# DarlingHang/st-nerf

Measured on NVIDIA H100. Metric: rays/sec, higher is better.
Workload: dtype f32 via fp16x3 split products (wgmma), f32 accumulate

## Files before the change

### st-nerf_b200/csrc/api.cu

```cuda
#include <algorithm>
#include <new>
#include <stdlib.h>
#include <string.h>
#include <vector>
#include "common.cuh"
#include "mlp_tc.cuh"

namespace stnerf {
thread_local char g_cuda_err[512] = "";
std::atomic<unsigned long long> g_launches{0};
}

using namespace stnerf;

namespace {

struct SpaceNetDev {
  float* blob = nullptr;
  SpaceNetW w{};
  TcNet tc{};
  bool loaded = false;
};
struct MotionNetDev {
  float* blob = nullptr;
// ... 4 lines not shown

}

struct stnerf_ctx {
  stnerf_model_desc desc{};
  int l = 0, num_sms = 0, device = 0, precision = 0, chunk_rays = 65536;
  SpaceNetDev space[2][STNERF_MAX_LAYERS];
  MotionNetDev motion[STNERF_MAX_LAYERS];
  stnerf_scene scene{};
  DevScene dscene{};
  bool have_scene = false;
  int cap_n1 = 0, cap_s2 = 0;
  long long last_chunk_rays = 0;
  int last_n1 = 0, last_s2 = 0;
  bool last_reuse = false;
  float *t_coarse = nullptr, *raw_coarse = nullptr, *t_fine = nullptr, *raw_fine = nullptr, *xyz = nullptr;
  float *xyz_coarse = nullptr, *z_new = nullptr;
  uint8_t* src_map = nullptr;
  bool no_reuse = false;
  float* cbuf = nullptr;
  uint8_t* mask_ws = nullptr;
  int *hit = nullptr, *counts = nullptr, *lerp_flags = nullptr;
  size_t ws_bytes = 0;
  float *h_rays = nullptr, *h_out = nullptr;
  uint8_t* h_mask = nullptr;
  size_t h_rays_bytes = 0, h_out_bytes = 0, h_mask_bytes = 0;
  float *v_rays = nullptr, *v_img[2] = {nullptr, nullptr};
  size_t v_rays_bytes = 0, v_img_bytes[2] = {0, 0};
  cudaStream_t copy_in = nullptr, copy_out = nullptr;
  std::vector<cudaEvent_t> ev_pool;
  float* box_table = nullptr;
  int box_frames = 0;
  bool no_fuse = false;
  int* any_frac = nullptr;
  RayIdMap idmap{0, 0, 0};
  int rot_mode[STNERF_MAX_LAYERS] = {0};
  float rot_R[STNERF_MAX_LAYERS][9] = {}, rot_c[STNERF_MAX_LAYERS][3] = {};
  struct ProfRec { int cls; cudaEvent_t a, b; double points; int count_slot; int S; };
  bool prof_on = false;
  std::vector<ProfRec> prof;
  int* prof_counts = nullptr;
  int prof_chunks = 0;
};

namespace {
constexpr int PROF_MAX_CHUNKS = 1 << 16;
struct ProfScope {
  stnerf_ctx* c; int idx = -1; cudaStream_t st;
  ProfScope(stnerf_ctx* c_, int cls, double points, int count_slot, int S, cudaStream_t st_) : c(c_), st(st_) {
    if (!c->prof_on) return;
    stnerf_ctx::ProfRec r{cls, nullptr, nullptr, points, count_slot, S};
    if (cudaEventCreate(&r.a) != cudaSuccess || cudaEventCreate(&r.b) != cudaSuccess) return;
    cudaEventRecord(r.a, st);
    c->prof.push_back(r);
    idx = (int)c->prof.size() - 1;
  }
  ~ProfScope() { if (idx >= 0) cudaEventRecord(c->prof[idx].b, st); }
};
}

static void free_ws(stnerf_ctx* c) {
  cudaFree(c->t_coarse); cudaFree(c->raw_coarse); cudaFree(c->t_fine); cudaFree(c->raw_fine); cudaFree(c->xyz);
  cudaFree(c->xyz_coarse); cudaFree(c->z_new); cudaFree(c->src_map);
  c->xyz_coarse = c->z_new = nullptr; c->src_map = nullptr;
  cudaFree(c->cbuf); c->cbuf = nullptr;
  cudaFree(c->mask_ws); cudaFree(c->hit); cudaFree(c->counts); cudaFree(c->lerp_flags);
// ... 53 lines not shown
    case STNERF_OK: return "ok";
    case STNERF_EINVAL: return "invalid argument";
    case STNERF_ENODEVICE: return "no usable CUDA device (needs sm_90)";
    case STNERF_ECUDA: return "CUDA runtime error (see stnerf_last_cuda_error)";
    case STNERF_ENOWEIGHTS: return "network weights not loaded";
    case STNERF_ENOMEM: return "out of device memory";
    default: return "unknown error";
  }
}
const char* stnerf_last_cuda_error(void) { return g_cuda_err; }
uint64_t stnerf_launch_count(void) { return g_launches.load(); }

int stnerf_create(stnerf_handle* out, const stnerf_model_desc* d) {
  if (!out || !d || d->n_layers < 2 || d->n_layers > STNERF_MAX_LAYERS) return STNERF_EINVAL;
  if (d->precision < 0 || d->precision > STNERF_PREC_TC_3XF16_CF || d->chunk_rays < 0) return STNERF_EINVAL;
  if ((long long)d->chunk_rays * STNERF_MAX_S >= (1LL << 31)) return STNERF_EINVAL;
  int ndev = 0;
  if (cudaGetDeviceCount(&ndev) != cudaSuccess || ndev == 0) { cudaGetLastError(); return STNERF_ENODEVICE; }
  int dev = 0;
  STNERF_CUDA(cudaGetDevice(&dev));
  cudaDeviceProp prop;
  STNERF_CUDA(cudaGetDeviceProperties(&prop, dev));
  if (prop.major != 9 || prop.minor != 0) return STNERF_ENODEVICE;
  stnerf_ctx* c = new (std::nothrow) stnerf_ctx();
  if (!c) return STNERF_ENOMEM;
  c->desc = *d;
  c->l = d->n_layers;
  c->device = dev;
  c->num_sms = prop.multiProcessorCount;
  c->precision = d->precision;
  c->chunk_rays = d->chunk_rays > 0 ? d->chunk_rays : 65536;
  if (const char* e = getenv("STNERF_NO_FUSE")) c->no_fuse = (e[0] == '1');
  if (const char* e = getenv("STNERF_NO_REUSE")) c->no_reuse = (e[0] == '1');
  if (cudaMalloc((void**)&c->any_frac, 4) != cudaSuccess) { delete c; return STNERF_ENOMEM; }
  *out = c;
  return STNERF_OK;
}

void stnerf_destroy(stnerf_handle c) {
  if (!c) return;
  cudaDeviceSynchronize();
  free_ws(c);
  for (int f = 0; f < 2; ++f)
    for (int i = 0; i < STNERF_MAX_LAYERS; ++i) { cudaFree(c->space[f][i].blob); tc_free(c->space[f][i].tc); }
  for (int i = 0; i < STNERF_MAX_LAYERS; ++i) { cudaFree(c->motion[i].blob); tc_free(c->motion[i].tc); }
  cudaFree(c->h_rays); cudaFree(c->h_out); cudaFree(c->h_mask); cudaFree(c->any_frac);
  cudaFree(c->v_rays); cudaFree(c->v_img[0]); cudaFree(c->v_img[1]); cudaFree(c->box_table);
  if (c->copy_in) cudaStreamDestroy(c->copy_in);
  if (c->copy_out) cudaStreamDestroy(c->copy_out);
  for (cudaEvent_t e : c->ev_pool) cudaEventDestroy(e);
  if (c->prof_counts) cudaFreeHost(c->prof_counts);
  delete c;
}

int stnerf_set_precision(stnerf_handle c, int precision) {
  if (!c || precision < 0 || precision > STNERF_PREC_TC_3XF16_CF) return STNERF_EINVAL;
  c->precision = precision;
  return STNERF_OK;
}

int stnerf_reserve(stnerf_handle c, int n1, int n2) {
  if (!c || n1 < 3 || n1 > STNERF_MAX_N1 || n2 < 0 || n1 + n2 > STNERF_MAX_S) return STNERF_EINVAL;
  return ensure_ws(c, n1, n1 + n2);
}
size_t stnerf_workspace_bytes(stnerf_handle c) { return c ? c->ws_bytes : 0; }

// ... 246 lines not shown
    if (n > 0 && cap > 0) STNERF_CUDA(cudaMallocAsync((void**)&buf, (size_t)n * cap * stride * sizeof(float), st));
    return STNERF_OK;
  }
  int rotate(const float* rays, long long m, LayerRays& lr) {
    for (int i = 0; i < STNERF_MAX_LAYERS; ++i) lr.p[i] = rays;
    for (int k = 0; k < n; ++k) {
      float* dst = buf + (size_t)k * cap * stride;
      const int rc = launch_rotate_rays(rays, m, stride, rot[k], dst, st);
      if (rc) return rc;
      lr.p[layer[k]] = dst;
    }
    return STNERF_OK;
  }
  ~RotatedRays() { if (buf) cudaFreeAsync(buf, st); }
};

static void fill_edit(PointSrc& s, const stnerf_scene& sc, int layer, bool fine) {
  s.shift_on = sc.shift_on[layer];
  s.scale_on = fine ? sc.scale_fine_on[layer] : sc.scale_coarse_on[layer];
  for (int a = 0; a < 3; ++a) { s.shift[a] = sc.shift[layer][a]; s.pivot[a] = sc.pivot[a]; }
  s.scale = sc.scale[layer];
  if (!s.scale_on) s.scale = 1.0f;
}

static int run_spacenet(stnerf_ctx* c, const PointSrc& src, SpaceNetDev& net, float* raw, float* rgb, float* sigma,
                        cudaStream_t st, int count_slot = -1, const FuseCoarse* fuse = nullptr, bool fine_pass = false) {
  if (!net.loaded) return STNERF_ENOWEIGHTS;
  ProfScope ps(c, 0, (double)src.n_slots * src.S, count_slot, src.S, st);
  if (c->precision == STNERF_PREC_FP32_SIMT)
    return launch_spacenet_simt(src, net.w, raw, 0, rgb, sigma, c->num_sms, st);
  if (src.mode == SRC_EXPLICIT) {
    float* cb = nullptr;
    STNERF_CUDA(cudaMallocAsync((void**)&cb, (size_t)std::max<long long>(src.n_slots, 1) * 128 * sizeof(float), st));
    const int rc = tc_launch_spacenet(src, net.tc, c->precision, cb, raw, rgb, sigma, c->num_sms, st, nullptr, fine_pass);
    STNERF_CUDA(cudaFreeAsync(cb, st));
    return rc;
  }
  return tc_launch_spacenet(src, net.tc, c->precision, c->cbuf, raw, rgb, sigma, c->num_sms, st, fuse, fine_pass);
}
static int run_motionnet(stnerf_ctx* c, const PointSrc& src, MotionNetDev& net, const int* lerp_flag, int lerp_force,
                         float* xyz_out, float* flow_out, cudaStream_t st, int count_slot = -1) {
  if (!net.loaded) return STNERF_ENOWEIGHTS;
  ProfScope ps(c, 1, (double)src.n_slots * src.S, count_slot, src.S, st);
  if (c->precision == STNERF_PREC_FP32_SIMT)
    return launch_motionnet_simt(src, net.w, lerp_flag, lerp_force, xyz_out, flow_out, c->num_sms, st);
  return tc_launch_motionnet(src, net.tc, c->precision, lerp_flag, lerp_force, xyz_out, flow_out, c->num_sms, st);
}

static int run_nets(stnerf_ctx* c, const LayerRays& rays, long long n, int ray_stride, bool fine, int S, cudaStream_t st,
                    int chunk_slot, const FuseCoarse* fuse = nullptr, bool want_raw = true, float* coarse_imgs = nullptr,
                    long long plane = 0, int reuse_n1 = 0) {
  const long long R = c->chunk_rays;
  const float* tbuf = fine ? c->t_fine : c->t_coarse;
  float* rawbuf = fine ? c->raw_fine : c->raw_coarse;
  const long long tl = R * (fine ? c->cap_s2 : c->cap_n1);
  for (int i = 0; i < c->l; ++i) {
    if (i > 0 && !c->scene.shown[i]) continue;
    PointSrc s;
    memset(&s, 0, sizeof(s));
    s.mode = SRC_MARCH;
    s.rays = rays.p[i]; s.ray_stride = ray_stride;
    s.t = tbuf + i * tl;
    s.S = S; s.layer = c->scene.shared_frame_id ? 0 : i;
    s.pos_stride = 3; s.time_stride = 1;
    fill_edit(s, c->scene, i, fine);
    float* raw = want_raw ? rawbuf + (size_t)i * tl * 4 : nullptr;
    FuseCoarse f;
    memset(&f, 0, sizeof(f));
    if (fuse) {
      f = *fuse;
      f.on = 1; f.layer = i; f.is_bkgd = (i == 0);
      f.t_fine = c->t_fine + (size_t)i * R * c->cap_s2;
      f.z_new = fuse->z_new ? c->z_new + (size_t)i * R * c->cap_s2 : nullptr;
      f.src_map = fuse->z_new ? c->src_map + (size_t)i * R * c->cap_s2 : nullptr;
      f.u = fuse->u ? fuse->u + (size_t)i * fuse->n_total * fuse->n2 : nullptr;
      f.img = coarse_imgs ? coarse_imgs + (size_t)(1 + i) * plane : nullptr;
    }
    int rc;
    if (i == 0) {
// ... 863 lines not shown
```

### st-nerf_b200/csrc/mlp_tc.cu

```cuda
#include <cuda_fp16.h>
#include <string.h>
#include <type_traits>
#include <vector>
#include "mlp_tc.cuh"
#include "resample.cuh"

namespace stnerf {

namespace {

constexpr int TILE_M = 128;
constexpr int ABLOCK = 16384;
constexpr int STAGE_BYTES = 16384;
constexpr int NTHREADS = 384;
constexpr int MATH_WG0 = 1, N_MATH_WARPS = 8;
constexpr int MAX_STAGE = 8;
constexpr int REGS_WG0 = 56, REGS_MATH = 224;
static_assert(128 * REGS_WG0 + 256 * REGS_MATH <= 384 * 168, "register file");
constexpr int BAR_WFULL = 0, BAR_WEMPTY = 8, BAR_RAWFULL = 16, BAR_RAWEMPTY = 18;
constexpr int MISC_ROWS = 256;
constexpr int MISC_PART = MISC_ROWS + 128 * 24;
constexpr int MISC_CDF = MISC_PART + 2048;
constexpr int MISC_TOTAL = MISC_CDF + 512;

__device__ __forceinline__ uint32_t smem_u32(const void* p) { return (uint32_t)__cvta_generic_to_shared(p); }

__device__ __forceinline__ void mbar_init(uint32_t bar, uint32_t count) {
  asm volatile("mbarrier.init.shared::cta.b64 [%0], %1;" ::"r"(bar), "r"(count) : "memory");
}
__device__ __forceinline__ void mbar_arrive(uint32_t bar) {
  asm volatile("mbarrier.arrive.shared::cta.b64 _, [%0];" ::"r"(bar) : "memory");
}
__device__ __forceinline__ void mbar_arrive_if(uint32_t bar, bool pred) {
  asm volatile("{\n\t.reg .pred p;\n\tsetp.ne.b32 p, %1, 0;\n\t@p mbarrier.arrive.shared::cta.b64 _, [%0];\n\t}" ::"r"(bar), "r"((uint32_t)pred)
               : "memory");
}
__device__ __forceinline__ void mbar_expect_tx(uint32_t bar, uint32_t bytes) {
  asm volatile("mbarrier.arrive.expect_tx.shared::cta.b64 _, [%0], %1;" ::"r"(bar), "r"(bytes) : "memory");
}
__device__ __forceinline__ void mbar_wait(uint32_t bar, uint32_t parity) {
  asm volatile(
      "{\n\t.reg .pred p;\n\t.reg .u32 c;\n\t"
      "mov.u32 c, 0;\n"
      "WAIT_%=:\n\t"
      "mbarrier.try_wait.parity.shared::cta.b64 p, [%0], %1;\n\t"
      "@p bra.uni DONE_%=;\n\t"
      "add.u32 c, c, 1;\n\t"
      "setp.gt.u32 p, c, 67108864;\n\t"
      "@p trap;\n\t"
      "bra.uni WAIT_%=;\n"
      "DONE_%=:\n\t}" ::"r"(bar), "r"(parity)
      : "memory");
}
__device__ __forceinline__ void bulk_g2s(uint32_t dst, const void* src, uint32_t bytes, uint32_t bar) {
  asm volatile("cp.async.bulk.shared::cluster.global.mbarrier::complete_tx::bytes [%0], [%1], %2, [%3];" ::"r"(dst),
               "l"(src), "r"(bytes), "r"(bar)
               : "memory");
}
__device__ __forceinline__ void fence_proxy_async() { asm volatile("fence.proxy.async.shared::cta;" ::: "memory"); }
template <int R>
__device__ __forceinline__ void setmaxnreg_dec() { asm volatile("setmaxnreg.dec.sync.aligned.u32 %0;" ::"n"(R)); }
template <int R>
__device__ __forceinline__ void setmaxnreg_inc() { asm volatile("setmaxnreg.inc.sync.aligned.u32 %0;" ::"n"(R)); }
__device__ __forceinline__ void wg_bar_sync(int wg) { asm volatile("bar.sync %0, 128;" ::"r"(1 + wg) : "memory"); }

__device__ __forceinline__ void load_stage_elect(uint32_t dst, const void* src, uint32_t bytes, uint32_t bar) {
  asm volatile(
      "{\n\t.reg .pred pe;\n\t"
      "elect.sync _|pe, 0xffffffff;\n\t"
      "@pe mbarrier.arrive.expect_tx.shared::cta.b64 _, [%3], %2;\n\t"
      "@pe cp.async.bulk.shared::cluster.global.mbarrier::complete_tx::bytes [%0], [%1], %2, [%3];\n\t}" ::"r"(dst),
      "l"(src), "r"(bytes), "r"(bar)
      : "memory");
}

__device__ __forceinline__ uint64_t desc_sw128(uint32_t saddr) {
  return (uint64_t)((saddr >> 4) & 0x3FFF) | ((uint64_t)1 << 16) | ((uint64_t)(1024 >> 4) << 32) | ((uint64_t)1 << 62);
}
__device__ __forceinline__ uint64_t desc_sw64(uint32_t saddr) {
  return (uint64_t)((saddr >> 4) & 0x3FFF) | ((uint64_t)1 << 16) | ((uint64_t)(512 >> 4) << 32) | ((uint64_t)2 << 62);
}
__device__ __forceinline__ void wgmma_fence() { asm volatile("wgmma.fence.sync.aligned;" ::: "memory"); }
__device__ __forceinline__ void wgmma_commit() { asm volatile("wgmma.commit_group.sync.aligned;" ::: "memory"); }
template <int N>
// ... 108 lines not shown
  static constexpr int LO_STRIDE = 2 * ABLOCK;
  static constexpr int ENC_LO_STRIDE = 2 * ABLOCK;
  static constexpr int n_stage = 8, stage_bytes = 8192;
  static constexpr int ring_base = 4 * ABLOCK, misc_base = ring_base + n_stage * stage_bytes, smem_total = misc_base + MISC_TOTAL;
  __host__ __device__ static constexpr int n_out(int) { return 128; }
  __host__ __device__ static constexpr int act_chunks(int l) { return l == 0 ? 0 : 2; }
  __host__ __device__ static constexpr int enc_chunks(int l) { return l == 0 ? 2 : 0; }
  __host__ __device__ static constexpr bool enc_first(int) { return false; }
};
static_assert(Sched<NET_SPACE>::n_stage <= MAX_STAGE && Sched<NET_MOTION>::n_stage <= MAX_STAGE, "barrier slots");

enum { A_HI = 0, A_LO = 1, A_HI_LO = 2 };
template <int A>
struct WStep {
  static constexpr int a = A;
  uint32_t offset;
  uint32_t sub;
};
template <int NET>
struct WSched {
  using S = Sched<NET>;
  __host__ __device__ static constexpr int n_chunks(int l) { return S::act_chunks(l) + S::enc_chunks(l); }
  __host__ __device__ static constexpr uint32_t stage_bytes(int l) { return (uint32_t)S::n_out(l) * 64; }
  __host__ __device__ static constexpr size_t layer_bytes(int l) { return (size_t)n_chunks(l) * 2  * 2  * stage_bytes(l); }
  __host__ __device__ static constexpr int chunk_at(int l, int c) {
    return S::enc_first(l) ? (c == 0 ? S::act_chunks(l) : c - 1) : c;
  }
  static constexpr bool enc_first_valid() {
    for (int l = 0; l < S::N_LAYERS; ++l)
      if (S::enc_first(l) && (S::act_chunks(l) == 0 || S::enc_chunks(l) == 0)) return false;
    return true;
  }
  static_assert(enc_first_valid(), "enc_first(l) needs activation chunks and an encoding chunk to reorder");
  template <bool LOFIRST, class C, class F>
  __device__ __forceinline__ static void for_each_step(int l, bool split, C&& chunk, F&& f) {
    const int nact = S::act_chunks(l), nch = nact + S::enc_chunks(l);
    const uint32_t bytes = stage_bytes(l);
    auto at = [&](const auto& a, int c, uint32_t sub, uint32_t lo_stage, auto op) {
      f(a, WStep<decltype(op)::value>{(2 * (2 * (uint32_t)c + sub) + lo_stage) * bytes, sub});
    };
    using HI = std::integral_constant<int, A_HI>;
    using LO = std::integral_constant<int, A_LO>;
    using HI_LO = std::integral_constant<int, A_HI_LO>;
    if (!LOFIRST || !split) {
      for (int c = 0; c < nch; ++c) {
        const auto a = chunk(chunk_at(l, c));
        for (uint32_t sub = 0; sub < 2; ++sub) {
          if (split) { at(a, c, sub, 1u, HI()); at(a, c, sub, 0u, HI_LO()); }
          else at(a, c, sub, 0u, HI());
        }
      }
    } else {
      for (int c = 0; c < nch; ++c) {
        const auto a = chunk(chunk_at(l, c));
        for (uint32_t sub = 0; sub < 2; ++sub) { at(a, c, sub, 1u, HI()); at(a, c, sub, 0u, LO()); }
      }
      for (int c = 0; c < nch; ++c) {
        const auto a = chunk(chunk_at(l, c));
        for (uint32_t sub = 0; sub < 2; ++sub) at(a, c, sub, 0u, HI());
      }
    }
  }
};

template <int NET>
__host__ __device__ constexpr size_t stream_bytes_per_tile() {
  size_t n = 0;
  for (int l = 0; l < Sched<NET>::N_LAYERS; ++l) n += WSched<NET>::layer_bytes(l);
  return n;
}

struct TcParams {
  FuseCoarse fuse;
  PointSrc src;
  const uint8_t* wstream;
  const float* aux;
  const float* cbuf;
  int exact;
  int single_last;
  int lo_first;
  float* raw;
  float* rgb_out;
  float* sigma_out;
  float* xyz_out;
  float* flow_out;
  const int* lerp_flag;
  int lerp_force;
};

constexpr int AUX_BIAS = 0, AUX_WSIG = 8 * 256, AUX_BSIG = AUX_WSIG + 256, AUX_WOUT = AUX_BSIG + 4,
              AUX_BOUT = AUX_WOUT + 3 * 128, AUX_FLOATS = AUX_BOUT + 4;


struct Pt { float x, y, z, tm; int out_index; int cidx; };

__device__ __forceinline__ Pt fetch_pt(const PointSrc& s, long long p, long long n_points) {
  Pt q;
  q.x = q.y = q.z = q.tm = 0.f;
  q.out_index = -1;
  q.cidx = 0;
  if (p >= n_points) return q;
  if (s.mode == SRC_EXPLICIT) {
    const float* pp = s.pos + p * s.pos_stride;
    q.x = pp[0]; q.y = pp[1]; q.z = pp[2];
    if (s.times) q.tm = s.times[p * s.time_stride];
    q.out_index = (int)p;
    q.cidx = (int)p;
    return q;
  }
  const long long slot = p / s.S;
  const int k = (int)(p - slot * s.S);
  const long long ray = s.hit ? (long long)s.hit[slot] : slot;
  const float* rp = s.rays + ray * s.ray_stride;
// ... 163 lines not shown
          if (F.apply_thr && v < F.thr) v = 0.0f;
        }
        t[s] = tk;
        sg[s] = v;
      }
      const float* up = F.u ? F.u + ray * n2 : nullptr;
      const uint64_t seed = F.seed;
      const uint32_t stream = 64u + (uint32_t)F.layer;
      const unsigned long long gid = F.idmap(F.ray_base + ray);
      rs::LayerOut lo;
      rs::composite_resample_ray<2, NZ>(
          t, sg, n1, n2, F.boarder,
          [rp, lane](int s) {
            const float4 v = rp[s * 32 + lane];
            return make_float3(__fdiv_rn(1.0f, __fadd_rn(1.0f, expf(-v.x))), __fdiv_rn(1.0f, __fadd_rn(1.0f, expf(-v.y))),
                               __fdiv_rn(1.0f, __fadd_rn(1.0f, expf(-v.z))));
          },
          [up, seed, stream, gid](int jj) { return up ? up[jj] : philox_uniform(seed, stream, gid, (uint32_t)jj); },
          cdf, F.t_fine + ray * (n1 + n2), lane, lo, F.z_new ? F.z_new + ray * n2 : nullptr,
          F.z_new ? F.src_map + ray * (n1 + n2) : nullptr);
      if (F.img && lane < 5) {
        const long long rg = F.ray_base + ray;
        const float v = lane == 0 ? lo.pix[0] : lane == 1 ? lo.pix[1] : lane == 2 ? lo.pix[2] : lane == 3 ? lo.pix[3] : lo.pix[4];
        if (F.pixels) F.img[rg * 5 + lane] = v;
        else if (lane < 3) F.img[rg * 3 + lane] = v;
        else F.img[(long long)lane * F.n_total + rg] = v;
      }
    }
    __syncwarp();
    if (lane == 0) mbar_arrive(bar_empty);
  }
}

template <int NET, int N, bool LOFIRST>
__device__ __forceinline__ void mma_layer(float (&acc)[128], const uint32_t (&alo)[64], int l, bool sp, uint32_t sbase,
                                          uint32_t a_row, uint32_t bars, uint32_t& cnt, int lane) {
  using S = Sched<NET>;
  using W = WSched<NET>;
  constexpr uint32_t NST = S::n_stage;
#pragma unroll
  for (int i = 0; i < N / 2; ++i) acc[i] = 0.f;
  acc_fence<N / 2>(acc);
  wgmma_fence();
  const int nact = S::act_chunks(l);
  int pend = -1;
  auto release = [&](int s) {
    __syncwarp();
    mbar_arrive_if(bars + 8u * (uint32_t)(BAR_WEMPTY + s), lane == 0);
  };
  auto a_block = [&](int ch) {
    uint32_t hi, lo = 0;
    int z = -1;
    if (ch < nact) {
      hi = sbase + S::act_base + ch * ABLOCK + a_row;
      if constexpr (S::lo_in_regs) z = ch;
      else lo = hi + S::LO_STRIDE;
    } else {
      hi = sbase + S::enc_base + (ch - nact) * ABLOCK + a_row;
      lo = hi + S::ENC_LO_STRIDE;
    }
    return make_int3((int)hi, (int)lo, z);
  };
  W::template for_each_step<LOFIRST>(l, sp, a_block, [&](const int3& a, auto st) {
    const uint32_t hi = (uint32_t)a.x + 64u * st.sub, lo = (uint32_t)a.y + 64u * st.sub;
    const uint32_t s = cnt % NST, n = cnt / NST;
    mbar_wait(bars + 8u * (BAR_WFULL + s), n & 1);
    const uint32_t w = sbase + S::ring_base + s * S::stage_bytes;
    auto mma_lo = [&]() {
      if (S::lo_in_regs && a.z >= 0) {
        const int q = 2 * a.z + (int)st.sub;
#pragma unroll
        for (int i = 0; i < 8; ++i)
          if (q == i) {
#pragma unroll
            for (int ks = 0; ks < 2; ++ks) wgmma_k16_rs<N>(acc, &alo[8 * i + 4 * ks], desc_sw64(w + ks * 32));
          }
      } else {
#pragma unroll
        for (int ks = 0; ks < 2; ++ks) wgmma_k16<N>(acc, desc_sw128(lo + ks * 32), desc_sw64(w + ks * 32));
      }
    };
    if constexpr (decltype(st)::a == A_LO) {
      mma_lo();
    } else {
#pragma unroll
      for (int ks = 0; ks < 2; ++ks) wgmma_k16<N>(acc, desc_sw128(hi + ks * 32), desc_sw64(w + ks * 32));
      if constexpr (decltype(st)::a == A_HI_LO) mma_lo();
    }
    wgmma_commit();
    wgmma_wait<1>();
    if (pend >= 0) release(pend);
    pend = (int)s;
    ++cnt;
  });
  wgmma_wait<0>();
  acc_fence<N / 2>(acc);
  release(pend);
}

template <int NET, int N, bool SIGMA>
__device__ __forceinline__ void epi_hidden(const float (&acc)[128], const float* __restrict__ bias, const float* __restrict__ wsig,
                                           uint8_t* smem, int r0, int cq, bool lo_too, float& sig0, float& sig1,
                                           uint32_t (&alo)[64]) {
  using S = Sched<NET>;
#pragma unroll
  for (int j = 0; j < N / 8; ++j) {
    const int col = 8 * j + cq;
    const float2 b = __ldg(reinterpret_cast<const float2*>(bias + col));
    const float v00 = fmaxf(acc[4 * j] + b.x, 0.f), v01 = fmaxf(acc[4 * j + 1] + b.y, 0.f);
    const float v10 = fmaxf(acc[4 * j + 2] + b.x, 0.f), v11 = fmaxf(acc[4 * j + 3] + b.y, 0.f);
    if (SIGMA) {
      const float2 w = __ldg(reinterpret_cast<const float2*>(wsig + col));
      sig0 = fmaf(v00, w.x, sig0); sig0 = fmaf(v01, w.y, sig0);
      sig1 = fmaf(v10, w.x, sig1); sig1 = fmaf(v11, w.y, sig1);
    }
    uint8_t* blk = smem + S::act_base + (col >> 6) * ABLOCK;
    const uint32_t o0 = sw128_offset(r0, col & 63), o1 = sw128_offset(r0 + 8, col & 63);
    const uint32_t h0 = pack_f16x2(v00, v01), h1 = pack_f16x2(v10, v11);
    *reinterpret_cast<uint32_t*>(blk + o0) = h0;
    *reinterpret_cast<uint32_t*>(blk + o1) = h1;
    const float2 f0 = unpack_f16x2(h0), f1 = unpack_f16x2(h1);
    const uint32_t l0 = pack_f16x2(v00 - f0.x, v01 - f0.y), l1 = pack_f16x2(v10 - f1.x, v11 - f1.y);
    if constexpr (S::lo_in_regs) {
      alo[2 * j] = l0;
      alo[2 * j + 1] = l1;
    } else if (lo_too) {
      *reinterpret_cast<uint32_t*>(blk + S::LO_STRIDE + o0) = l0;
      *reinterpret_cast<uint32_t*>(blk + S::LO_STRIDE + o1) = l1;
    }
// ... 4 lines not shown
  v += __shfl_xor_sync(0xffffffffu, v, 1);
  v += __shfl_xor_sync(0xffffffffu, v, 2);
  return v;
}

template <int NET, bool LOFIRST>
__global__ void __launch_bounds__(NTHREADS, 1) mlp_tc_kernel(const __grid_constant__ TcParams P) {
  using S = Sched<NET>;
  extern __shared__ __align__(1024) uint8_t smem[];
  const uint32_t sbase = smem_u32(smem);
  if ((sbase & 1023u) != 0) {
    if (threadIdx.x == 0) printf("stnerf mlp_tc: dynamic shared memory base %u is not 1024-byte aligned\n", sbase);
    __trap();
  }
  const uint32_t bars = sbase + S::misc_base;
  auto BAR = [bars](int i) { return bars + 8u * (uint32_t)i; };
  Pt* s_rows = reinterpret_cast<Pt*>(smem + S::misc_base + MISC_ROWS);
  float* s_part = reinterpret_cast<float*>(smem + S::misc_base + MISC_PART);

  const int tid = threadIdx.x, lane = tid & 31;
  const int warp = __shfl_sync(0xffffffffu, tid >> 5, 0);
  const int wgi = __shfl_sync(0xffffffffu, tid >> 7, 0);
  const bool exact = P.exact != 0;
  const bool single_last = P.single_last != 0;
  auto split = [&](int l) { return exact && !(single_last && l == S::N_LAYERS - 1); };
  const long long n_points = src_num_points(P.src);
  const long long n_tiles = (n_points + TILE_M - 1) / TILE_M;
  constexpr uint32_t NST = S::n_stage;
  if (tid == 0) {
    for (int i = 0; i < MAX_STAGE; ++i) { mbar_init(BAR(BAR_WFULL + i), 1); mbar_init(BAR(BAR_WEMPTY + i), N_MATH_WARPS); }
    for (int j = 0; j < 2; ++j) {
      mbar_init(BAR(BAR_RAWFULL + j), 4);
      mbar_init(BAR(BAR_RAWEMPTY + j), 1);
    }
    asm volatile("fence.mbarrier_init.release.cluster;" ::: "memory");
  }
  __syncthreads();

  if (wgi < MATH_WG0) {
    if constexpr (S::lo_in_regs) setmaxnreg_dec<REGS_WG0>();
    if (warp == 0) {
      using W = WSched<NET>;
      uint32_t cnt = 0;
      for (long long tile = blockIdx.x; tile < n_tiles; tile += gridDim.x) {
        const uint8_t* layer = P.wstream;
        for (int l = 0; l < S::N_LAYERS; ++l) {
          W::template for_each_step<LOFIRST>(l, split(l), [](int) { return 0; }, [&](int, auto st) {
            const uint32_t s = cnt % NST, n = cnt / NST;
            mbar_wait(BAR(BAR_WEMPTY + s), (n & 1) ^ 1);
            load_stage_elect(sbase + S::ring_base + s * S::stage_bytes, layer + st.offset, W::stage_bytes(l), BAR(BAR_WFULL + s));
            ++cnt;
          });
          layer += W::layer_bytes(l);
        }
      }
    } else if (NET == NET_SPACE && (warp == 2 || warp == 3)) {
      if (P.fuse.on) {
        const int j = warp - 2;
        float* cdf = reinterpret_cast<float*>(smem + S::misc_base + MISC_CDF) + j * 64;
        if (P.fuse.n2 <= 128)
          fused_composite_loop<4>(P, s_part, cdf, BAR(BAR_RAWFULL + j), BAR(BAR_RAWEMPTY + j), n_tiles, j, lane);
        else
          fused_composite_loop<8>(P, s_part, cdf, BAR(BAR_RAWFULL + j), BAR(BAR_RAWEMPTY + j), n_tiles, j, lane);
      }
    }
  } else {
    if constexpr (S::lo_in_regs) setmaxnreg_inc<REGS_MATH>();
    const int wg = wgi - MATH_WG0;
    const int wt = tid & 127;
    const int erow = wg * 64 + (wt & 63), ehalf = wt >> 6;
    const int r0 = wg * 64 + (wt >> 5) * 16 + (lane >> 2);
    const int cq = 2 * (lane & 3);
    const uint32_t a_row = (uint32_t)wg * 8u * 1024u;
    const float* bias_all = P.aux + AUX_BIAS;
    const bool lerp = (NET == NET_MOTION) && (P.lerp_force >= 0 ? (P.lerp_force != 0) : (P.lerp_flag && *P.lerp_flag != 0));
    const bool fused = (NET == NET_SPACE) && P.fuse.on;
    uint32_t cnt = 0, tile_no = 0;
    float acc[128];
    uint32_t alo[64];
#pragma unroll
    for (int i = 0; i < 64; ++i) alo[i] = 0u;
    for (long long tile = blockIdx.x; tile < n_tiles; tile += gridDim.x, ++tile_no) {
      wg_bar_sync(wg);
      const Pt cur = fetch_pt(P.src, tile * TILE_M + erow, n_points);
      if (ehalf == 0) s_rows[erow] = cur;
      float carry[2] = {0.f, 0.f};
      if (NET == NET_MOTION) {
        uint8_t* enc = smem + S::enc_base + ehalf * ABLOCK;
        for (int c = (ehalf == 0 ? 48 : 40); c < 64; c += 8) {
          const uint32_t off = sw128_offset(erow, c);
          *reinterpret_cast<uint4*>(enc + off) = make_uint4(0, 0, 0, 0);
          *reinterpret_cast<uint4*>(enc + S::ENC_LO_STRIDE + off) = make_uint4(0, 0, 0, 0);
        }
      }
      encode_piece<NET, 0>(smem, cur, erow, ehalf, exact, lerp, carry);
      encode_piece<NET, 1>(smem, cur, erow, ehalf, exact, lerp, carry);
      if (NET == NET_MOTION) encode_piece<NET, 2>(smem, cur, erow, ehalf, exact, lerp, carry);
      float sig0 = 0.f, sig1 = 0.f;
      for (int l = 0; l < S::N_LAYERS; ++l) {
        fence_proxy_async();
        wg_bar_sync(wg);
        const bool last = (l == S::N_LAYERS - 1);
        if (!last) {
          mma_layer<NET, (NET == NET_SPACE ? 256 : 128), LOFIRST>(acc, alo, l, split(l), sbase, a_row, bars, cnt, lane);
          if (NET == NET_SPACE && l == 6)
            epi_hidden<NET, 256, true>(acc, bias_all + l * 256, P.aux + AUX_WSIG, smem, r0, cq, split(l + 1), sig0, sig1, alo);
          else
            epi_hidden<NET, (NET == NET_SPACE ? 256 : 128), false>(acc, bias_all + l * 256, nullptr, smem, r0, cq, split(l + 1), sig0,
                                                                  sig1, alo);
          continue;
        }
        mma_layer<NET, 128, LOFIRST>(acc, alo, l, split(l), sbase, a_row, bars, cnt, lane);
        const Pt p0 = s_rows[r0], p1 = s_rows[r0 + 8];
        const float* b0 = (NET == NET_SPACE) ? (P.cbuf + (size_t)p0.cidx * 128) : bias_all + l * 256;
        const float* b1 = (NET == NET_SPACE) ? (P.cbuf + (size_t)p1.cidx * 128) : bias_all + l * 256;
        float d0[3] = {0.f, 0.f, 0.f}, d1[3] = {0.f, 0.f, 0.f};
#pragma unroll
        for (int j = 0; j < 16; ++j) {
          const int col = 8 * j + cq;
          const float2 ba = __ldg(reinterpret_cast<const float2*>(b0 + col));
          const float2 bb = __ldg(reinterpret_cast<const float2*>(b1 + col));
          const float v00 = fmaxf(acc[4 * j] + ba.x, 0.f), v01 = fmaxf(acc[4 * j + 1] + ba.y, 0.f);
          const float v10 = fmaxf(acc[4 * j + 2] + bb.x, 0.f), v11 = fmaxf(acc[4 * j + 3] + bb.y, 0.f);
#pragma unroll
          for (int o = 0; o < 3; ++o) {
            const float2 w = __ldg(reinterpret_cast<const float2*>(P.aux + AUX_WOUT + o * 128 + col));
            d0[o] = fmaf(v00, w.x, d0[o]); d0[o] = fmaf(v01, w.y, d0[o]);
            d1[o] = fmaf(v10, w.x, d1[o]); d1[o] = fmaf(v11, w.y, d1[o]);
          }
        }
#pragma unroll
        for (int o = 0; o < 3; ++o) { d0[o] = quad_sum(d0[o]) + P.aux[AUX_BOUT + o]; d1[o] = quad_sum(d1[o]) + P.aux[AUX_BOUT + o]; }
        if (NET == NET_SPACE) { sig0 = quad_sum(sig0) + P.aux[AUX_BSIG]; sig1 = quad_sum(sig1) + P.aux[AUX_BSIG]; }
        if (fused) {
          if (tile_no > 0) mbar_wait(BAR(BAR_RAWEMPTY + wg), (tile_no - 1) & 1);
          if ((lane & 3) == 0) {
            reinterpret_cast<float4*>(s_part)[r0] = make_float4(d0[0], d0[1], d0[2], sig0);
            reinterpret_cast<float4*>(s_part)[r0 + 8] = make_float4(d1[0], d1[1], d1[2], sig1);
          }
          __syncwarp();
          if (lane == 0) mbar_arrive(BAR(BAR_RAWFULL + wg));
        }
        if ((lane & 3) == 0) {
#pragma unroll
          for (int h = 0; h < 2; ++h) {
            const Pt& p = h ? p1 : p0;
            const float* o = h ? d1 : d0;
            const float sg = h ? sig1 : sig0;
            if (p.out_index < 0) continue;
            const int oi = p.out_index;
            if (NET == NET_SPACE) {
              if (P.raw) reinterpret_cast<float4*>(P.raw)[oi] = make_float4(o[0], o[1], o[2], sg);
              if (P.rgb_out) { P.rgb_out[3 * (size_t)oi] = o[0]; P.rgb_out[3 * (size_t)oi + 1] = o[1]; P.rgb_out[3 * (size_t)oi + 2] = o[2]; }
              if (P.sigma_out) P.sigma_out[oi] = sg;
            } else {
              const long long pidx = tile * TILE_M + r0 + 8 * h;
              if (P.flow_out) { P.flow_out[3 * pidx] = o[0]; P.flow_out[3 * pidx + 1] = o[1]; P.flow_out[3 * pidx + 2] = o[2]; }
              if (P.xyz_out) {
                P.xyz_out[3 * pidx] = __fadd_rn(p.x, o[0]);
                P.xyz_out[3 * pidx + 1] = __fadd_rn(p.y, o[1]);
                P.xyz_out[3 * pidx + 2] = __fadd_rn(p.z, o[2]);
              }
            }
          }
        }
      }
    }
  }
}

constexpr int HB_SLOTS = 8;
__global__ void __launch_bounds__(128) head_bias_kernel(PointSrc src, const float* __restrict__ w_tail ,
                                                        const float* __restrict__ b1, int use_time,
                                                        float* __restrict__ cbuf) {
  __shared__ float s_enc[HB_SLOTS][48];
  const long long n_slots = src.count ? (long long)(*src.count) : src.n_slots;
  const int nk = PE_DIR + (use_time ? PE_TIME : 0);
  const int tid = threadIdx.x;
  float w[48];
#pragma unroll
  for (int k = 0; k < 48; ++k) w[k] = (k < nk) ? __ldg(w_tail + k * 128 + tid) : 0.f;
  const float bias = __ldg(b1 + tid);
  for (long long s0 = (long long)blockIdx.x * HB_SLOTS; s0 < n_slots; s0 += (long long)gridDim.x * HB_SLOTS) {
    __syncthreads();
    for (int e = tid; e < HB_SLOTS * 48; e += 128) {
      const int sl = e / 48, j = e - sl * 48;
      const long long slot = s0 + sl;
      float v = 0.f;
      if (slot < n_slots && j < nk) {
        float d[3], tm;
        if (src.mode == SRC_EXPLICIT) {
          d[0] = src.dirs[3 * slot]; d[1] = src.dirs[3 * slot + 1]; d[2] = src.dirs[3 * slot + 2];
          tm = src.times ? src.times[slot * src.time_stride] : 0.f;
        } else {
          const long long ray = src.hit ? (long long)src.hit[slot] : slot;
          const float* rp = src.rays + ray * src.ray_stride;
          d[0] = rp[3]; d[1] = rp[4]; d[2] = rp[5];
          tm = rp[6 + src.layer];
// ... 267 lines not shown
  cudaFree(dA); cudaFree(dB); cudaFree(dD);
  float worst = 0.f;
  double signed_rel = 0.0;
  for (int m = 0; m < 128; ++m)
    for (int n = 0; n < 256; ++n) {
      double ref = 0;
      for (int k = 0; k < 64; ++k) ref += (double)Af[m * 64 + k] * Bf[n * 64 + k];
      ref *= reps;
      worst = fmaxf(worst, fabsf((float)(ref - (double)D[m * 256 + n])));
      if (ref != 0.0) signed_rel += ((double)D[m * 256 + n] - ref) / fabs(ref);
    }
  *max_err_host = worst;
  if (mean_signed_rel_host) *mean_signed_rel_host = (float)(signed_rel / (128.0 * 256.0));
  return STNERF_OK;
}
int tc_selftest(float* max_err_host) { return tc_selftest_accum(1, max_err_host, nullptr); }

template <int NET, bool LOFIRST>
static int launch_tc_variant(const TcParams& P, int num_sms, cudaStream_t st) {
  using S = Sched<NET>;
  auto kern = mlp_tc_kernel<NET, LOFIRST>;
  STNERF_CUDA(cudaFuncSetAttribute(kern, cudaFuncAttributeMaxDynamicSharedMemorySize, S::smem_total));
  kern<<<num_sms, NTHREADS, S::smem_total, st>>>(P);
  STNERF_LAUNCH_CHECK();
  return STNERF_OK;
}

template <int NET>
static int launch_tc(const TcParams& P, int num_sms, cudaStream_t st) {
  return P.lo_first ? launch_tc_variant<NET, true>(P, num_sms, st) : launch_tc_variant<NET, false>(P, num_sms, st);
}

bool tc_can_fuse_coarse(int n1, int n2) { return n1 == 64 && n2 >= 1 && n2 <= 256; }

int tc_launch_spacenet(const PointSrc& src, const TcNet& net, int precision, float* cbuf, float* raw,
                       float* rgb_out, float* sigma_out, int num_sms, cudaStream_t st, const FuseCoarse* fuse, bool fine_pass) {
  if (!net.blob || !net.w_tail) return STNERF_ENOWEIGHTS;
  if (!cbuf) return STNERF_EINVAL;
  PointSrc hs = src;
  if (src.mode == SRC_EXPLICIT) hs.count = nullptr;
  const long long slots_hint = src.count ? src.n_slots_cap : src.n_slots;
  long long blocks = (slots_hint + HB_SLOTS - 1) / HB_SLOTS;
  if (blocks < 1) blocks = 1;
  if (blocks > (long long)num_sms * 8) blocks = (long long)num_sms * 8;
  head_bias_kernel<<<(int)blocks, 128, 0, st>>>(hs, net.w_tail, net.aux + AUX_BIAS + 7 * 256, net.use_time, cbuf);
  STNERF_LAUNCH_CHECK();
  TcParams P;
  memset(&P, 0, sizeof(P));
  P.src = src; P.wstream = (const uint8_t*)net.blob; P.aux = net.aux; P.cbuf = cbuf;
  P.exact = precision == STNERF_PREC_TC_3XF16 || precision == STNERF_PREC_TC_MIXED || precision == STNERF_PREC_TC_3XF16_CF;
  P.single_last = precision == STNERF_PREC_TC_MIXED;
  P.raw = raw; P.rgb_out = rgb_out; P.sigma_out = sigma_out; P.lerp_force = 0;
  P.lo_first = precision == STNERF_PREC_TC_3XF16_CF && !fine_pass;
  if (fuse && fuse->on) {
    if (src.mode == SRC_EXPLICIT || src.S != 64 || !tc_can_fuse_coarse(fuse->n1, fuse->n2) || !fuse->t_fine) return STNERF_EINVAL;
    P.fuse = *fuse;
  }
  return launch_tc<NET_SPACE>(P, num_sms, st);
}

int tc_launch_motionnet(const PointSrc& src, const TcNet& net, int precision, const int* lerp_flag_dev,
                        int lerp_force, float* xyz_out, float* flow_out, int num_sms, cudaStream_t st) {
  if (!net.blob) return STNERF_ENOWEIGHTS;
  TcParams P;
  memset(&P, 0, sizeof(P));
  P.src = src; P.wstream = (const uint8_t*)net.blob; P.aux = net.aux;
  P.exact = precision == STNERF_PREC_TC_3XF16 || precision == STNERF_PREC_TC_MIXED || precision == STNERF_PREC_TC_3XF16_CF;
  P.xyz_out = xyz_out; P.flow_out = flow_out; P.lerp_flag = lerp_flag_dev; P.lerp_force = lerp_force;
  P.lo_first = precision == STNERF_PREC_TC_3XF16_CF;
  return launch_tc<NET_MOTION>(P, num_sms, st);
}

}
```

### st-nerf_b200/csrc/mlp_tc.cuh

```cuda
#pragma once
#include "common.cuh"

namespace stnerf {

struct FuseCoarse {
  int on;
  int n1, n2, layer, is_bkgd;
  const float* u;
  uint64_t seed;
  RayIdMap idmap;
  long long ray_base;
  float* t_fine;
  float* z_new;
  uint8_t* src_map;
  float* img;
  long long n_total;
  int pixels;
  float near_plane, thr, boarder;
  int apply_thr;
};

struct TcNet {
  void* blob = nullptr;
  size_t blob_bytes = 0;
  float* aux = nullptr;
  float* w_tail = nullptr;
  int use_time = 0;
};

int tc_pack_spacenet(TcNet& net, const float* blob_host, bool use_time);
int tc_pack_motionnet(TcNet& net, const float* blob_host);
void tc_free(TcNet& net);
size_t tc_stream_bytes(bool is_space);
size_t tc_aux_floats();
size_t tc_tail_floats(bool is_space);
int tc_export(const TcNet& net, bool is_space, uint8_t* stream_host, float* aux_host, float* tail_host);
int tc_import(TcNet& net, bool is_space, int use_time, const uint8_t* stream_host, const float* aux_host, const float* tail_host);
int tc_selftest(float* max_err_host);
int tc_selftest_accum(int reps, float* max_err_host, float* mean_signed_rel_host);
int tc_launch_spacenet(const PointSrc& src, const TcNet& net, int precision, float* cbuf, float* raw, float* rgb_out,
                       float* sigma_out, int num_sms, cudaStream_t st, const FuseCoarse* fuse = nullptr, bool fine_pass = false);
bool tc_can_fuse_coarse(int n1, int n2);
int tc_launch_motionnet(const PointSrc& src, const TcNet& net, int precision, const int* lerp_flag_dev, int lerp_force,
                        float* xyz_out, float* flow_out, int num_sms, cudaStream_t st);

}
```

Before: 748,200.

## Stagger math warpgroups per layer with mbarrier hand-off to offset wgmma phases

Adds a per-layer hand-off mbarrier pair so the second math warpgroup waits until the lead warpgroup has issued a configurable number of weight-stream steps (default 3) before it starts its own wgmma chain. The point is to desynchronise the two consumer warpgroups so their epilogues and MMA bursts interleave instead of contending at the same time. It also adds an optional compile-time clock64 timeline probe. The cost is an extra wait per layer per tile for the trailing warpgroup, plus the risk of longer stalls on the weight ring if the lead gets too far ahead.

```diff
diff --git a/st-nerf_b200/csrc/api.cu b/st-nerf_b200/csrc/api.cu
--- a/st-nerf_b200/csrc/api.cu
+++ b/st-nerf_b200/csrc/api.cu
@@ -60,6 +60,7 @@
   float* box_table = nullptr;
   int box_frames = 0;
   bool no_fuse = false;
+  int mlp_stagger = 3;
   int* any_frac = nullptr;
   RayIdMap idmap{0, 0, 0};
   int rot_mode[STNERF_MAX_LAYERS] = {0};
@@ -179,6 +180,7 @@
   c->chunk_rays = d->chunk_rays > 0 ? d->chunk_rays : 65536;
   if (const char* e = getenv("STNERF_NO_FUSE")) c->no_fuse = (e[0] == '1');
   if (const char* e = getenv("STNERF_NO_REUSE")) c->no_reuse = (e[0] == '1');
+  if (const char* e = getenv("STNERF_MLP_STAGGER")) c->mlp_stagger = std::min(std::max(atoi(e), 0), tc_max_stagger());
   if (cudaMalloc((void**)&c->any_frac, 4) != cudaSuccess) { delete c; return STNERF_ENOMEM; }
   *out = c;
   return STNERF_OK;
@@ -491,11 +493,13 @@
   if (src.mode == SRC_EXPLICIT) {
     float* cb = nullptr;
     STNERF_CUDA(cudaMallocAsync((void**)&cb, (size_t)std::max<long long>(src.n_slots, 1) * 128 * sizeof(float), st));
-    const int rc = tc_launch_spacenet(src, net.tc, c->precision, cb, raw, rgb, sigma, c->num_sms, st, nullptr, fine_pass);
+    const int rc = tc_launch_spacenet(src, net.tc, c->precision, c->mlp_stagger, cb, raw, rgb, sigma, c->num_sms, st, nullptr,
+                                      fine_pass);
     STNERF_CUDA(cudaFreeAsync(cb, st));
     return rc;
   }
-  return tc_launch_spacenet(src, net.tc, c->precision, c->cbuf, raw, rgb, sigma, c->num_sms, st, fuse, fine_pass);
+  return tc_launch_spacenet(src, net.tc, c->precision, c->mlp_stagger, c->cbuf, raw, rgb, sigma, c->num_sms, st, fuse,
+                            fine_pass);
 }
 static int run_motionnet(stnerf_ctx* c, const PointSrc& src, MotionNetDev& net, const int* lerp_flag, int lerp_force,
                          float* xyz_out, float* flow_out, cudaStream_t st, int count_slot = -1) {
@@ -503,7 +507,8 @@
   ProfScope ps(c, 1, (double)src.n_slots * src.S, count_slot, src.S, st);
   if (c->precision == STNERF_PREC_FP32_SIMT)
     return launch_motionnet_simt(src, net.w, lerp_flag, lerp_force, xyz_out, flow_out, c->num_sms, st);
-  return tc_launch_motionnet(src, net.tc, c->precision, lerp_flag, lerp_force, xyz_out, flow_out, c->num_sms, st);
+  return tc_launch_motionnet(src, net.tc, c->precision, c->mlp_stagger, lerp_flag, lerp_force, xyz_out, flow_out, c->num_sms,
+                             st);
 }
 
 static int run_nets(stnerf_ctx* c, const LayerRays& rays, long long n, int ray_stride, bool fine, int S, cudaStream_t st,
diff --git a/st-nerf_b200/csrc/mlp_tc.cu b/st-nerf_b200/csrc/mlp_tc.cu
--- a/st-nerf_b200/csrc/mlp_tc.cu
+++ b/st-nerf_b200/csrc/mlp_tc.cu
@@ -17,7 +17,8 @@
 constexpr int MAX_STAGE = 8;
 constexpr int REGS_WG0 = 56, REGS_MATH = 224;
 static_assert(128 * REGS_WG0 + 256 * REGS_MATH <= 384 * 168, "register file");
-constexpr int BAR_WFULL = 0, BAR_WEMPTY = 8, BAR_RAWFULL = 16, BAR_RAWEMPTY = 18;
+constexpr int BAR_WFULL = 0, BAR_WEMPTY = 8, BAR_RAWFULL = 16, BAR_RAWEMPTY = 18, BAR_HAND = 20;
+constexpr int MAX_STAGGER = 6;
 constexpr int MISC_ROWS = 256;
 constexpr int MISC_PART = MISC_ROWS + 128 * 24;
 constexpr int MISC_CDF = MISC_PART + 2048;
@@ -50,6 +51,22 @@
       "@p trap;\n\t"
       "bra.uni WAIT_%=;\n"
       "DONE_%=:\n\t}" ::"r"(bar), "r"(parity)
+      : "memory");
+}
+__device__ __forceinline__ void mbar_wait_if(uint32_t bar, uint32_t parity, bool pred) {
+  asm volatile(
+      "{\n\t.reg .pred p;\n\t.reg .u32 c;\n\t"
+      "setp.eq.u32 p, %2, 0;\n\t"
+      "@p bra.uni DONE_%=;\n\t"
+      "mov.u32 c, 0;\n"
+      "WAIT_%=:\n\t"
+      "mbarrier.try_wait.parity.shared::cta.b64 p, [%0], %1;\n\t"
+      "@p bra.uni DONE_%=;\n\t"
+      "add.u32 c, c, 1;\n\t"
+      "setp.gt.u32 p, c, 67108864;\n\t"
+      "@p trap;\n\t"
+      "bra.uni WAIT_%=;\n"
+      "DONE_%=:\n\t}" ::"r"(bar), "r"(parity), "r"((uint32_t)pred)
       : "memory");
 }
 __device__ __forceinline__ void bulk_g2s(uint32_t dst, const void* src, uint32_t bytes, uint32_t bar) {
@@ -224,6 +241,20 @@
     return true;
   }
   static_assert(enc_first_valid(), "enc_first(l) needs activation chunks and an encoding chunk to reorder");
+  __host__ __device__ static constexpr int n_steps(int l, bool split, bool lofirst) {
+    return n_chunks(l) * 2 * (!split ? 1 : lofirst ? 3 : 2);
+  }
+  static constexpr bool handoff_cannot_lap() {
+    for (int l = 0; l < S::N_LAYERS; ++l) {
+      const int next = (l + 1) % S::N_LAYERS;
+      for (int sp = 0; sp < 2; ++sp)
+        for (int sn = 0; sn < 2; ++sn)
+          if (n_steps(l, sp, false) + n_steps(next, sn, false) + 1 <= S::n_stage) return false;
+    }
+    return true;
+  }
+  static_assert(handoff_cannot_lap(), "the hand-off barriers can alias: use more of them");
+  static_assert(MAX_STAGGER < S::n_stage, "the lead must fit inside the ring");
   template <bool LOFIRST, class C, class F>
   __device__ __forceinline__ static void for_each_step(int l, bool split, C&& chunk, F&& f) {
     const int nact = S::act_chunks(l), nch = nact + S::enc_chunks(l);
@@ -271,6 +302,7 @@
   int exact;
   int single_last;
   int lo_first;
+  int stagger;
   float* raw;
   float* rgb_out;
   float* sigma_out;
@@ -500,12 +532,36 @@
   }
 }
 
+constexpr int TL_CTAS = 132, TL_TILE0 = 4, TL_TILES = 8, TL_SLOTS = 32, TL_START = 0, TL_ENC = 1, TL_LAYER = 2;
+#ifdef STNERF_MLP_TIMELINE
+__device__ unsigned long long g_timeline[TL_CTAS * TL_TILES * 2 * TL_SLOTS];
+#endif
+struct TileClock {
+#ifdef STNERF_MLP_TIMELINE
+  unsigned long long* row = nullptr;
+  __device__ __forceinline__ void at(uint32_t tile_no, int wg) {
+    const uint32_t t = tile_no - TL_TILE0;
+    row = (blockIdx.x < TL_CTAS && t < TL_TILES) ? g_timeline + ((blockIdx.x * TL_TILES + t) * 2 + wg) * TL_SLOTS : nullptr;
+  }
+  __device__ __forceinline__ void stamp(int i, bool pred = true) const {
+    if (pred && row && (threadIdx.x & 127) == 0) row[i] = clock64();
+  }
+#else
+  __device__ __forceinline__ void at(uint32_t, int) {}
+  __device__ __forceinline__ void stamp(int, bool = true) const {}
+#endif
+};
+static_assert(TL_LAYER + 3 * Sched<NET_SPACE>::N_LAYERS <= TL_SLOTS, "timeline slots");
+
 template <int NET, int N, bool LOFIRST>
 __device__ __forceinline__ void mma_layer(float (&acc)[128], const uint32_t (&alo)[64], int l, bool sp, uint32_t sbase,
-                                          uint32_t a_row, uint32_t bars, uint32_t& cnt, int lane) {
+                                          uint32_t a_row, uint32_t bars, uint32_t& cnt, int lane, uint32_t hand,
+                                          uint32_t hand_par, bool hand_wait, uint32_t hand_sig, const TileClock& tl) {
   using S = Sched<NET>;
   using W = WSched<NET>;
   constexpr uint32_t NST = S::n_stage;
+  mbar_wait_if(hand, hand_par, hand_wait);
+  const uint32_t cnt0 = cnt;
 #pragma unroll
   for (int i = 0; i < N / 2; ++i) acc[i] = 0.f;
   acc_fence<N / 2>(acc);
@@ -556,6 +612,8 @@
       if constexpr (decltype(st)::a == A_HI_LO) mma_lo();
     }
     wgmma_commit();
+    mbar_arrive_if(hand, lane == 0 && cnt == hand_sig);
+    tl.stamp(TL_LAYER + 3 * l, cnt == cnt0);
     wgmma_wait<1>();
     if (pend >= 0) release(pend);
     pend = (int)s;
@@ -563,6 +621,7 @@
   });
   wgmma_wait<0>();
   acc_fence<N / 2>(acc);
+  tl.stamp(TL_LAYER + 3 * l + 1);
   release(pend);
 }
 
@@ -633,6 +692,7 @@
     for (int j = 0; j < 2; ++j) {
       mbar_init(BAR(BAR_RAWFULL + j), 4);
       mbar_init(BAR(BAR_RAWEMPTY + j), 1);
+      mbar_init(BAR(BAR_HAND + j), 4);
     }
     asm volatile("fence.mbarrier_init.release.cluster;" ::: "memory");
   }
@@ -667,6 +727,7 @@
     }
   } else {
     if constexpr (S::lo_in_regs) setmaxnreg_inc<REGS_MATH>();
+    using W = WSched<NET>;
     const int wg = wgi - MATH_WG0;
     const int wt = tid & 127;
     const int erow = wg * 64 + (wt & 63), ehalf = wt >> 6;
@@ -677,12 +738,17 @@
     const bool lerp = (NET == NET_MOTION) && (P.lerp_force >= 0 ? (P.lerp_force != 0) : (P.lerp_flag && *P.lerp_flag != 0));
     const bool fused = (NET == NET_SPACE) && P.fuse.on;
     uint32_t cnt = 0, tile_no = 0;
+    uint32_t n_hand = 0;
+    TileClock tl;
+    const bool lead = wg == 0;
     float acc[128];
     uint32_t alo[64];
 #pragma unroll
     for (int i = 0; i < 64; ++i) alo[i] = 0u;
     for (long long tile = blockIdx.x; tile < n_tiles; tile += gridDim.x, ++tile_no) {
       wg_bar_sync(wg);
+      tl.at(tile_no, wg);
+      tl.stamp(TL_START);
       const Pt cur = fetch_pt(P.src, tile * TILE_M + erow, n_points);
       if (ehalf == 0) s_rows[erow] = cur;
       float carry[2] = {0.f, 0.f};
@@ -697,21 +763,30 @@
       encode_piece<NET, 0>(smem, cur, erow, ehalf, exact, lerp, carry);
       encode_piece<NET, 1>(smem, cur, erow, ehalf, exact, lerp, carry);
       if (NET == NET_MOTION) encode_piece<NET, 2>(smem, cur, erow, ehalf, exact, lerp, carry);
+      tl.stamp(TL_ENC);
       float sig0 = 0.f, sig1 = 0.f;
       for (int l = 0; l < S::N_LAYERS; ++l) {
         fence_proxy_async();
         wg_bar_sync(wg);
         const bool last = (l == S::N_LAYERS - 1);
+        const int dl = min(P.stagger, W::n_steps(l, split(l), LOFIRST) - 1);
+        const uint32_t hand = BAR(BAR_HAND + (n_hand & 1)), hand_par = (n_hand >> 1) & 1;
+        const bool hand_wait = !lead && dl > 0;
+        const uint32_t hand_sig = (lead && dl > 0) ? cnt + (uint32_t)dl - 1 : 0xffffffffu;
+        ++n_hand;
         if (!last) {
-          mma_layer<NET, (NET == NET_SPACE ? 256 : 128), LOFIRST>(acc, alo, l, split(l), sbase, a_row, bars, cnt, lane);
+          mma_layer<NET, (NET == NET_SPACE ? 256 : 128), LOFIRST>(acc, alo, l, split(l), sbase, a_row, bars, cnt, lane, hand,
+                                                                 hand_par, hand_wait, hand_sig, tl);
           if (NET == NET_SPACE && l == 6)
             epi_hidden<NET, 256, true>(acc, bias_all + l * 256, P.aux + AUX_WSIG, smem, r0, cq, split(l + 1), sig0, sig1, alo);
           else
             epi_hidden<NET, (NET == NET_SPACE ? 256 : 128), false>(acc, bias_all + l * 256, nullptr, smem, r0, cq, split(l + 1), sig0,
                                                                   sig1, alo);
+          tl.stamp(TL_LAYER + 3 * l + 2);
           continue;
         }
-        mma_layer<NET, 128, LOFIRST>(acc, alo, l, split(l), sbase, a_row, bars, cnt, lane);
+        mma_layer<NET, 128, LOFIRST>(acc, alo, l, split(l), sbase, a_row, bars, cnt, lane, hand, hand_par, hand_wait, hand_sig,
+                                     tl);
         const Pt p0 = s_rows[r0], p1 = s_rows[r0 + 8];
         const float* b0 = (NET == NET_SPACE) ? (P.cbuf + (size_t)p0.cidx * 128) : bias_all + l * 256;
         const float* b1 = (NET == NET_SPACE) ? (P.cbuf + (size_t)p1.cidx * 128) : bias_all + l * 256;
@@ -765,6 +840,7 @@
             }
           }
         }
+        tl.stamp(TL_LAYER + 3 * l + 2);
       }
     }
   }
@@ -1098,11 +1174,12 @@
 }
 
 bool tc_can_fuse_coarse(int n1, int n2) { return n1 == 64 && n2 >= 1 && n2 <= 256; }
-
-int tc_launch_spacenet(const PointSrc& src, const TcNet& net, int precision, float* cbuf, float* raw,
+int tc_max_stagger() { return MAX_STAGGER; }
+
+int tc_launch_spacenet(const PointSrc& src, const TcNet& net, int precision, int stagger, float* cbuf, float* raw,
                        float* rgb_out, float* sigma_out, int num_sms, cudaStream_t st, const FuseCoarse* fuse, bool fine_pass) {
   if (!net.blob || !net.w_tail) return STNERF_ENOWEIGHTS;
-  if (!cbuf) return STNERF_EINVAL;
+  if (!cbuf || stagger < 0 || stagger > MAX_STAGGER) return STNERF_EINVAL;
   PointSrc hs = src;
   if (src.mode == SRC_EXPLICIT) hs.count = nullptr;
   const long long slots_hint = src.count ? src.n_slots_cap : src.n_slots;
@@ -1117,6 +1194,7 @@
   P.exact = precision == STNERF_PREC_TC_3XF16 || precision == STNERF_PREC_TC_MIXED || precision == STNERF_PREC_TC_3XF16_CF;
   P.single_last = precision == STNERF_PREC_TC_MIXED;
   P.raw = raw; P.rgb_out = rgb_out; P.sigma_out = sigma_out; P.lerp_force = 0;
+  P.stagger = stagger;
   P.lo_first = precision == STNERF_PREC_TC_3XF16_CF && !fine_pass;
   if (fuse && fuse->on) {
     if (src.mode == SRC_EXPLICIT || src.S != 64 || !tc_can_fuse_coarse(fuse->n1, fuse->n2) || !fuse->t_fine) return STNERF_EINVAL;
@@ -1125,16 +1203,32 @@
   return launch_tc<NET_SPACE>(P, num_sms, st);
 }
 
-int tc_launch_motionnet(const PointSrc& src, const TcNet& net, int precision, const int* lerp_flag_dev,
+int tc_launch_motionnet(const PointSrc& src, const TcNet& net, int precision, int stagger, const int* lerp_flag_dev,
                         int lerp_force, float* xyz_out, float* flow_out, int num_sms, cudaStream_t st) {
   if (!net.blob) return STNERF_ENOWEIGHTS;
+  if (stagger < 0 || stagger > MAX_STAGGER) return STNERF_EINVAL;
   TcParams P;
   memset(&P, 0, sizeof(P));
   P.src = src; P.wstream = (const uint8_t*)net.blob; P.aux = net.aux;
   P.exact = precision == STNERF_PREC_TC_3XF16 || precision == STNERF_PREC_TC_MIXED || precision == STNERF_PREC_TC_3XF16_CF;
   P.xyz_out = xyz_out; P.flow_out = flow_out; P.lerp_flag = lerp_flag_dev; P.lerp_force = lerp_force;
   P.lo_first = precision == STNERF_PREC_TC_3XF16_CF;
+  P.stagger = stagger;
   return launch_tc<NET_MOTION>(P, num_sms, st);
 }
 
 }
+
+#ifdef STNERF_MLP_TIMELINE
+extern "C" int stnerf_mlp_timeline(unsigned long long* host, int* dims) {
+  using namespace stnerf;
+  if (dims) { dims[0] = TL_CTAS; dims[1] = TL_TILES; dims[2] = 2; dims[3] = TL_SLOTS; }
+  if (!host) return STNERF_OK;
+  STNERF_CUDA(cudaDeviceSynchronize());
+  STNERF_CUDA(cudaMemcpyFromSymbol(host, g_timeline, sizeof(g_timeline)));
+  void* dev = nullptr;
+  STNERF_CUDA(cudaGetSymbolAddress(&dev, g_timeline));
+  STNERF_CUDA(cudaMemset(dev, 0, sizeof(g_timeline)));
+  return STNERF_OK;
+}
+#endif
diff --git a/st-nerf_b200/csrc/mlp_tc.cuh b/st-nerf_b200/csrc/mlp_tc.cuh
--- a/st-nerf_b200/csrc/mlp_tc.cuh
+++ b/st-nerf_b200/csrc/mlp_tc.cuh
@@ -38,10 +38,12 @@
 int tc_import(TcNet& net, bool is_space, int use_time, const uint8_t* stream_host, const float* aux_host, const float* tail_host);
 int tc_selftest(float* max_err_host);
 int tc_selftest_accum(int reps, float* max_err_host, float* mean_signed_rel_host);
-int tc_launch_spacenet(const PointSrc& src, const TcNet& net, int precision, float* cbuf, float* raw, float* rgb_out,
-                       float* sigma_out, int num_sms, cudaStream_t st, const FuseCoarse* fuse = nullptr, bool fine_pass = false);
+int tc_launch_spacenet(const PointSrc& src, const TcNet& net, int precision, int stagger, float* cbuf, float* raw,
+                       float* rgb_out, float* sigma_out, int num_sms, cudaStream_t st, const FuseCoarse* fuse = nullptr,
+                       bool fine_pass = false);
 bool tc_can_fuse_coarse(int n1, int n2);
-int tc_launch_motionnet(const PointSrc& src, const TcNet& net, int precision, const int* lerp_flag_dev, int lerp_force,
-                        float* xyz_out, float* flow_out, int num_sms, cudaStream_t st);
+int tc_launch_motionnet(const PointSrc& src, const TcNet& net, int precision, int stagger, const int* lerp_flag_dev,
+                        int lerp_force, float* xyz_out, float* flow_out, int num_sms, cudaStream_t st);
+int tc_max_stagger();
 
 }
```

Result: no change. 751,100, median of 6 (+0.4%).
